# logannye/streaming-zero-knowledge-proofs

Hardware: AMD Instinct MI355X
Metric: STARK prove field-elements/sec (NTT+FRI+Merkle), 2^24 domain, 1/2/4/8 GPUs (higher is better)
Workload: dtype u64; 1 GPU; stark-v1 prove, T=2^21 rows (N=2^24 LDE domain), b=512, tau=8, trace resident in HBM when the timed region starts, proof bytes on the host (host_to_proof beside it: every proof uploads its own trace over PCIe); T=2097152, N=16777216, tau=8, b=512, proof_bytes=2301655, proofs_in_flight_per_gpu=3, upload_bytes_per_proof=69206016, parallelism=replicas x1, 3 independent proofs in flight per GPU

## Files before the change

### include/sezkp_stark.h

```cpp
#ifndef SEZKP_STARK_H
#define SEZKP_STARK_H

#include <stddef.h>
#include <stdint.h>

#ifdef __cplusplus
extern "C" {
#endif

#define SEZKP_ABI_VERSION 4u

#define SEZKP_OK 0
#define SEZKP_E_INVALID (-1)
#define SEZKP_E_DEVICE (-2)
#define SEZKP_E_NOMEM (-3)
#define SEZKP_E_DECODE (-4)
#define SEZKP_E_VERIFY (-5)

#define SEZKP_FLAG_STREAMING 1u

uint32_t sezkp_abi_version(void);
const char* sezkp_version(void);

typedef struct sezkp_buf {
// ... 51 lines not shown
                              size_t err_len);
int32_t sezkp_ctx_wait(sezkp_ctx* ctx, const uint8_t** data, size_t* len, char* err, size_t err_len);
void* sezkp_ctx_stream(const sezkp_ctx* ctx);
typedef struct sezkp_dict_plan_info {
  uint32_t col;
  uint32_t kind;
  uint32_t tape;
  int32_t K;
  uint32_t a;
  uint32_t delta;
  uint32_t R;
  uint32_t dR;
  int64_t min;
} sezkp_dict_plan_info;
int32_t sezkp_ctx_dict_plans(const sezkp_ctx* ctx, sezkp_dict_plan_info* out, int32_t max);

#define SEZKP_AIR_FAMILIES 5
typedef struct sezkp_air_family {
  uint64_t cells, rows, first_row;
  uint32_t first_tape, pad;
  uint64_t first_value;
} sezkp_air_family;
typedef struct sezkp_air_audit {
  uint64_t n_rows;
  uint32_t tau, pad;
  uint64_t rows_violating, first_violating, rows_rejectable, first_rejectable;
  sezkp_air_family fam[SEZKP_AIR_FAMILIES];
} sezkp_air_audit;
int32_t sezkp_ctx_air_audit(sezkp_ctx* ctx, sezkp_air_audit* out, uint8_t* violating_bits, uint8_t* rejectable_bits,
                            char* err, size_t err_len);
// ... 72 lines not shown
```

### streaming-zero-knowledge-proofs_amd/csrc/prover.cpp

```cpp
#include <hip/hip_runtime.h>
#include <stdio.h>
#include <stdlib.h>
#include <string.h>

#include <algorithm>
#include <chrono>
#include <condition_variable>
#include <map>
#include <memory>
#include <mutex>
#include <string>
#include <thread>
#include <vector>

#include "../../include/sezkp_stark.h"
#include "codec.h"
#include "comm.h"
#include "host_crypto.h"
#include "sezkp_internal.h"

using namespace sezkp;

namespace {

// ... 154 lines not shown
  int n_tab_cols = 0;
  uint64_t tab_units = 0;
  uint32_t* d_work = nullptr;
  int n_work = 0;
  uint32_t* d_pw_cols = nullptr;
  int n_pw_cols = 0;
  uint32_t* d_pw_chunks = nullptr;
  int n_pw_chunks = 0;
  DictCol* d_dcols = nullptr;
  int n_dict = 0;
  int64_t* d_dpart = nullptr;
  DictPlan* d_dplans = nullptr;
  std::vector<sezkp_dict_plan_info> dict_info;
  bool have_plans = false;
  uint32_t* d_dtabs = nullptr;
  uint32_t* d_dlev = nullptr;
  std::vector<uint32_t> dict_of;
  uint32_t* d_outer = nullptr;
  uint32_t* d_err = nullptr;
  uint64_t outer_stride = 0;
  uint32_t* d_colroots = nullptr;
  uint64_t* d_base = nullptr;
  ComposeTerms Tm{};
  uint64_t *d_dq_part = nullptr, *d_dq_rlo = nullptr, *d_dq_rhi = nullptr, *d_dq_rhk = nullptr;
  uint64_t* d_lde = nullptr;
  uint64_t* d_fri = nullptr;
  uint32_t* d_roots = nullptr;
  DevChal* d_chal = nullptr;
  DevChal* h_chal = nullptr;
  uint32_t* d_dict_of = nullptr;
// ... 165 lines not shown
    if (async) {
      {
        std::unique_lock<std::mutex> lk(async->mu);
        async->cv.wait(lk, [&] { return async->state != AsyncSlot::RUNNING; });
        async->stop = true;
      }
      async->cv.notify_all();
      if (async->th.joinable()) async->th.join();
    }
    if (st) (void)hipStreamSynchronize(st);
    if (st2) (void)hipStreamSynchronize(st2);
    if (stc) (void)hipStreamSynchronize(stc);
    free_all();
    release_spares();
    free_audit();
    if (h_audit) (void)hipHostFree(h_audit);
    for (auto& e : ev)
      if (e) (void)hipEventDestroy(e);
    for (auto& e : coll_ev) (void)hipEventDestroy(e);
    for (auto& e : kev)
      if (e) (void)hipEventDestroy(e);
    for (auto& e : oev)
      if (e) (void)hipEventDestroy(e);
    if (st2) (void)hipStreamSynchronize(st2);
    if (ev_fold) (void)hipEventDestroy(ev_fold);
    if (ev_tail) (void)hipEventDestroy(ev_tail);
    if (ev_expand) (void)hipEventDestroy(ev_expand);
    if (ev_cols) (void)hipEventDestroy(ev_cols);
    if (ev_qin) (void)hipEventDestroy(ev_qin);
    if (ev_qout) (void)hipEventDestroy(ev_qout);
// ... 238 lines not shown
      for (uint32_t j = k; j < nblk && v.step_start[j] < c1; j++)
        if (j == 0 || v.step_start[j] != v.step_start[j - 1]) inside++;
      if (ch < ch_lo || ch >= ch_hi) continue;
      if (inside <= 16) pw_chunks.push_back((uint32_t)ch);
      else dense_chunk[ch] = 1;
    }
  }
  for (int c = 0; c < ncols; c++) {
    if (use_dict && kind_dict(tm[c].kind)) continue;
    const bool pw = kind_piecewise(tm[c].kind);
    for (uint64_t ch = ch_lo; ch < ch_hi; ch++)
      if (!pw || dense_chunk[ch]) { work.push_back((uint32_t)c); work.push_back((uint32_t)ch); }
  }
  d_tmpl = dalloc<ColTemplate>(ncols);
  up(d_tmpl, tm.data(), tm.size());
  d_colroots = dalloc<uint32_t>((size_t)ncols * 8 + 16);
  d_err = d_colroots + (size_t)ncols * 8;
  HIP_OR_THROW(hipMemset(d_err, 0, 64));
  d_tabs = dalloc<uint32_t>(tab_nodes * 8 + 8);
  n_tab_cols = (int)tab_cols.size();
  d_tab_cols = dalloc<uint32_t>(tab_cols.size() + 1);
  up(d_tab_cols, tab_cols.data(), tab_cols.size());
  for (DictCol& h : dcols)
    if (tm[h.col].kind == 6)
      for (size_t i = 0; i < dcols.size(); i++)
        if (tm[dcols[i].col].kind == 3 && tm[dcols[i].col].tape == tm[h.col].tape) h.mv = (uint32_t)i;
  n_dict = (int)dcols.size();
  have_plans = false;
  dict_info.assign(dcols.size(), sezkp_dict_plan_info{});
  for (size_t i = 0; i < dcols.size(); i++) {
    dict_info[i].col = dcols[i].col;
    dict_info[i].kind = tm[dcols[i].col].kind;
    dict_info[i].tape = tm[dcols[i].col].tape;
  }
  d_dcols = dalloc<DictCol>(dcols.size() + 1);
  up(d_dcols, dcols.data(), dcols.size());
  d_dpart = dalloc<int64_t>(2 * dcols.size() * ((n + 4095) / 4096) + 2);
  d_dplans = dalloc<DictPlan>(dcols.size() + 1);
  d_dtabs = dalloc<uint32_t>(dcols.size() * DICT_LEVELS * DICT_CAP * 8 + 8);
  d_dlev = dalloc<uint32_t>(dcols.size() * (n >> COL_CHUNK_LOG2) * DLEV_NODES * 8 + 8);
  dict_of.assign(ncols, NO_DICT);
  for (size_t i = 0; i < dcols.size(); i++) dict_of[dcols[i].col] = (uint32_t)i;
  n_pw_cols = (int)pw_cols.size();
  d_pw_cols = dalloc<uint32_t>(pw_cols.size() + 1);
  up(d_pw_cols, pw_cols.data(), pw_cols.size());
  n_pw_chunks = (int)pw_chunks.size();
  d_pw_chunks = dalloc<uint32_t>(pw_chunks.size() + 1);
  up(d_pw_chunks, pw_chunks.data(), pw_chunks.size());
  n_work = (int)(work.size() / 2);
  d_work = dalloc<uint32_t>(work.size() + 2);
  up(d_work, work.data(), work.size());
  outer_stride = tree_stored_nodes(logChunks, 0);
  d_outer = dalloc<uint32_t>((size_t)ncols * outer_stride * 8);

// ... 149 lines not shown
    PL.nq = NUM_QUERIES;
    PL.k = k;
    PL.tau = tau;
    PL.open_bytes = 80 + 32 * (uint64_t)logn;
    PL.q_bytes = 16 + PL.open_per_q * PL.open_bytes;
    PL.fr_off = 8 + NUM_QUERIES * PL.q_bytes;
    PL.fq_off = PL.fr_off + 8 + 32 * (uint64_t)(k + 1);
    PL.fq_bytes = 8 + 8 * (uint64_t)(k + 1) + 8;
    for (int r = 0; r < k; r++) PL.fq_bytes += 2 * (16 + 32 * (uint64_t)(k - r));
    PL.tail_off = PL.fq_off + 8 + NUM_QUERIES * PL.fq_bytes;
    PL.total = PL.tail_off + 8 + 32;
    PL.base = dalloc<uint32_t>(PL.total / 4 + 2);
    h_proof = halloc<uint8_t>(hdr_bytes + PL.total);
    memcpy(h_proof, w.b.data(), hdr_bytes);
  }
  h_small = halloc<uint32_t>((size_t)(ncols + k + 2) * 8);
  d_chal = dalloc<DevChal>(1);
  h_chal = halloc<DevChal>(1);
  d_dict_of = dalloc<uint32_t>((size_t)ncols);
  up(d_dict_of, dict_of.data(), dict_of.size());
  if (k > FS_MAX_BETAS) throw Err{SEZKP_E_INVALID, "LDE domain too large for the challenge record"};
  release_spares();
  loaded = true;
}

void sezkp_ctx::alloc_slot(TraceSlot& t) {
  const size_t cells = (size_t)tau * n, nt = (size_t)tau * nblk;
  t.imv = dalloc<int8_t>(n);
  t.mv = dalloc<int8_t>(cells);
  t.wf = dalloc<uint8_t>(cells);
  t.ws = dalloc<uint16_t>(cells);
// ... 273 lines not shown
  const bool no_deep_poly = getenv("SEZKP_NO_DEEP_POLY") != nullptr;
  uint32_t dict_tab_cap = DICT_CAP;
  if (const char* cap = getenv("SEZKP_DICT_TAB_CAP")) {
    const long v = atol(cap);
    if (v >= 1 && v <= (long)DICT_CAP) dict_tab_cap = (uint32_t)v;
  }
  uint64_t dict_plan_rows = 0;
  if (const char* pr = getenv("SEZKP_TEST_DICT_PLAN_ROWS_LOG")) {
    long v = atol(pr);
    int lg = 0;
    while ((2ULL << lg) <= row_hi - row_lo) lg++;
    const long v_max = lg >= 16 ? 40 : 20 + (lg > 14 ? lg - 14 : 0);
    if (v > v_max) v = v_max;
    if (v >= COL_CHUNK_LOG2 && v <= 40) dict_plan_rows = 1ULL << v;
  }
  const int nguard = sharded ? comm->world : 1;
  auto check_guards = [&](const uint32_t* g_h, int ng) {
    for (int r = 0; r < ng; r++) {
      const uint32_t g = g_h[r];
      if (g) {
        const hipError_t me = hipMemsetAsync(d_err, 0, 64, st);
        if (me != hipSuccess) {
          broken = true;
          throw Err{SEZKP_E_DEVICE, std::string("guard word tripped (code ") + std::to_string(g) +
                                        ") and clearing it failed: " + hipGetErrorString(me) +
                                        "; the context is unusable"};
        }
      }
      const std::string who = " on rank " + std::to_string(sharded ? r : rank);
      if (g & GUARD_HEAD_RANGE) throw Err{SEZKP_E_INVALID, head_range_msg(who)};
// ... 13 lines not shown
  size_t nf = 0, no = 0;

  auto enqueue_A = [&]() {
    rec(0);
    ok(launch_expand(st, T, blk_lo, blk_cnt, d_err), "expand");
    rec(1);
    HIP_OR_THROW(hipEventRecord(ev_expand, st));
    HIP_OR_THROW(hipStreamWaitEvent(st2, ev_expand, 0));
    ok(launch_col_tables(st2, T, d_tmpl, d_tab_cols, n_tab_cols, tab_units, d_tabs, blk_lo, blk_cnt), "col_tables");
    ok(launch_col_commit(st2, T, d_tmpl, d_work, n_work, d_tabs, d_outer, outer_stride), "col_commit");
    ok(launch_col_commit_pw(st2, T, d_tmpl, d_pw_cols, n_pw_cols, d_pw_chunks, n_pw_chunks, d_tabs, d_outer,
                            outer_stride, d_err), "col_commit_pw");
    ok(launch_compose_terms(st2, T, Tm, row_lo, row_hi - row_lo), "compose_terms");
    HIP_OR_THROW(hipEventRecord(ev_cols, st2));
    ok(launch_dict_commit(st, T, d_tmpl, d_dcols, n_dict, d_dpart, d_dplans, d_dtabs, d_outer, outer_stride, row_lo,
                          row_hi - row_lo, d_dlev, dict_tab_cap, dict_plan_rows),
       "col_commit_dict");
    HIP_OR_THROW(hipStreamWaitEvent(st, ev_cols, 0));
    static const char* trip = getenv("SEZKP_DEBUG_TRIP_GUARD");
    if (trip && atoi(trip) == rank) HIP_OR_THROW(hipMemsetAsync(d_err, 0x7f, 1, st));
    if (sharded) {
      const size_t bytes = (size_t)(ch_hi - ch_lo) * 32;
      coll("col_chunk_roots", P1 * (bytes * ncols + 4), [&] {
        comm->group_start();
        for (int c = 0; c < ncols; c++) {
          uint32_t* lvl0 = d_outer + (size_t)c * outer_stride * 8;
          comm->allgather(lvl0 + ch_lo * 8, lvl0, bytes, st);
        }
        comm->allgather(d_err, d_err + 8, 4, st);
        comm->group_end();
      });
    }
    rec(2);
    TreeDev outer0{d_outer, d_colroots, logChunks, 0};
    ok(launch_tree_upper(st, &outer0, ncols, outer_stride, 8, 0), "col_outer");
    rec(3);
    HIP_OR_THROW(hipMemcpyAsync(h_small, d_colroots, (size_t)ncols * 32 + 4 * (gofs + nguard), hipMemcpyDeviceToHost,
                                st));
  };
  auto host_1 = [&]() {
    const uint32_t* colroots_h = h_small;
    check_guards(h_small + 8 * ncols + gofs, nguard);
    std::vector<uint8_t> colroots((const uint8_t*)colroots_h, (const uint8_t*)colroots_h + (size_t)ncols * 32);
    for (int c = 0; c < ncols; c++) memcpy(h_proof + root_pos[c], colroots.data() + 32 * c, 32);

    tr.absorb("manifest_root", mroot, 32);
    tr.absorb_u64("n", n);
    tr.absorb_u64("tau", tau);
    tr.absorb_u64("n_cols", (uint64_t)ncols);
    for (int c = 0; c < ncols; c++) tr.absorb("col_root", colroots.data() + 32 * c, 32);
    mark("tr_roots");
    auto ab = tr.challenge("alphas", 64);
    uint64_t a[8];
    for (int i = 0; i < 8; i++) a[i] = rd64(ab.data() + 8 * i) % GL_P_HOST;
    tr.absorb("masks", "masks", 5);
    tr.absorb_u64("n_masks", 1);
    tr.absorb_u64("deg", 4);
// ... 370 lines not shown
  for (int q = 0; q < NUM_QUERIES; q++) {
    const uint64_t at = PL.fq_off + 8 + q * PL.fq_bytes;
    put64(at, (uint64_t)k + 1);
    for (int r = 0; r <= k; r++) put64(at + 8 + 8 * r, pos[(size_t)q * (k + 1) + r]);
    put64(at + 8 + 8 * (uint64_t)(k + 1), (uint64_t)k);
  }
  memcpy(body + PL.tail_off, h_small + 8 * (k + 1), 8);
  memcpy(body + PL.tail_off + 8, mroot, 32);
  const size_t out = hdr_bytes + PL.total;
  const auto t_end = clk::now();
  host_ms[0] = std::chrono::duration<double, std::milli>(t_end - t_enter).count();
  host_ms[1] = t_sync;
  host_ms[2] = t_last;
  host_ms[3] = std::chrono::duration<double, std::milli>(t_end - t_ser).count();
  have_plans = true;
  return out;
}

extern "C" {

uint32_t sezkp_abi_version(void) { return SEZKP_ABI_VERSION; }
const char* sezkp_version(void) { return "sezkp-mi355x 0.1.0 (stark-v1, gfx950)"; }

void sezkp_buf_free(sezkp_buf* b) {
  if (b && b->data) {
    free(b->data);
    b->data = nullptr;
    b->len = 0;
  }
}
// ... 287 lines not shown
      hipMemcpy(pl.data(), ctx->d_dplans, (size_t)cnt * sizeof(DictPlan), hipMemcpyDeviceToHost) != hipSuccess) {
    (void)hipGetLastError();
    return SEZKP_E_DEVICE;
  }
  for (int32_t i = 0; i < cnt; i++) {
    sezkp_dict_plan_info& o = out[i];
    o = ctx->dict_info[(size_t)i];
    o.K = pl[i].K;
    o.a = pl[i].a;
    o.delta = pl[i].delta;
    o.R = pl[i].R;
    o.dR = pl[i].delta ? pl[i].dR : 0;
    o.min = pl[i].min;
  }
  return cnt;
}
int32_t sezkp_ctx_comm_stats(const sezkp_ctx* ctx, sezkp_comm_stat* out, int32_t max) {
  if (!ctx || !out || max <= 0) return 0;
  int32_t cnt = 0;
  for (const auto& c : ctx->coll_stats) {
    if (cnt >= max) break;
    sezkp_comm_stat& o = out[cnt++];
    memset(o.name, 0, sizeof o.name);
    strncpy(o.name, c.name, sizeof o.name - 1);
    o.bytes = c.bytes;
    float ms = 0;
    o.ms = hipEventElapsedTime(&ms, c.a, c.b) == hipSuccess ? ms : -1.0;
  }
  (void)hipGetLastError();
  return cnt;
// ... 450 lines not shown
```

### streaming-zero-knowledge-proofs_amd/csrc/sezkp_internal.h

```cpp
#pragma once
#include <hip/hip_runtime.h>
#include <stddef.h>
#include <stdint.h>

#include <vector>

namespace sezkp {

struct DevChal;
struct ComposeTerms;

struct NttTables {
  const uint64_t* hi;
  const uint64_t* lo;
  const uint64_t* p3_hi;
  const uint64_t* p3_lo;
  int K;
  int S;
};

struct NttPassArgs {
  uint64_t* a;
  const uint64_t* src;
  NttTables tw;
// ... 136 lines not shown
struct DictCol {
  uint32_t col;
  uint32_t mv;
  uint64_t tab;
};
struct DictPlan {
  int64_t min;
  uint32_t R;
  int32_t K;
  uint32_t pw[DICT_LEVELS];
  uint32_t delta;
  int64_t dmin;
  uint32_t dR;
  uint32_t a;
};
__host__ __device__ inline bool kind_dict(uint32_t kind) { return kind == 0 || (kind >= 3 && kind <= 6); }
constexpr int DICT_LANE_LOG = 6;
constexpr int DLEV_NODES = 30;
__host__ __device__ inline int dlev_base(int level) { return level == 6 ? 0 : level == 7 ? 16 : level == 8 ? 24 : 28; }
constexpr uint32_t NO_DICT = 0xFFFFFFFFu;
__host__ __device__ inline int dict_extra(int K) { return K >= 3 ? 2 : (K == 2 ? 1 : 0); }
constexpr int OPEN_REQ_WORDS = 5;

constexpr int LSTORE_FRI = 6;
constexpr int COL_CHUNK_LOG2 = 10;
struct ProofLayout {
  uint32_t* base;
  uint64_t open_bytes;
  uint64_t q_bytes;
  uint64_t fr_off, fq_off, fq_bytes, tail_off, total;
// ... 11 lines not shown
  uint64_t K3;
  uint64_t beta[FS_MAX_BETAS];
};

hipError_t launch_trace_image(hipStream_t st, const int8_t* raw_mv, const uint8_t* raw_hw, const uint16_t* raw_ws,
                              uint64_t n, int tau, int8_t* mv, uint8_t* wf, uint16_t* ws, uint64_t r0 = 0,
                              uint64_t r1 = ~0ull);
hipError_t launch_expand(hipStream_t st, const TraceDev& T, uint32_t blk_lo, uint32_t blk_cnt, uint32_t* d_err);
hipError_t launch_col_tables(hipStream_t st, const TraceDev& T, const ColTemplate* d_tmpl, const uint32_t* d_tab_cols,
                             int n_tab_cols, uint64_t tab_entries, uint32_t* tabs, uint32_t blk_lo, uint32_t blk_cnt);
hipError_t launch_col_commit(hipStream_t st, const TraceDev& T, const ColTemplate* d_tmpl, const uint32_t* d_work,
                             int nwork, const uint32_t* tabs, uint32_t* outer_nodes, uint64_t outer_stride_nodes);
hipError_t launch_dict_commit(hipStream_t st, const TraceDev& T, const ColTemplate* d_tmpl, const DictCol* d_dcols,
                              int ndict, int64_t* d_part, DictPlan* d_plans, uint32_t* d_dtabs, uint32_t* outer_nodes,
                              uint64_t outer_stride_nodes, uint64_t row0, uint64_t nrows, uint32_t* d_dlev,
                              uint32_t tab_cap = DICT_CAP, uint64_t plan_rows = 0);
hipError_t launch_dict_prepare(hipStream_t st, const TraceDev& T, const ColTemplate* d_tmpl, const DictCol* d_dcols,
                               int ndict, int64_t* d_part, DictPlan* d_plans, uint64_t row0, uint64_t nrows,
                               uint32_t tab_cap = DICT_CAP, uint64_t plan_rows = 0);
hipError_t launch_dict_levels(hipStream_t st, const ColTemplate* d_tmpl, const DictCol* d_dcols, int ndict,
                              const DictPlan* d_plans, uint32_t* d_dtabs, int lvl_lo, int lvl_hi);
hipError_t launch_dict_commit_cols(hipStream_t st, const TraceDev& T, const ColTemplate* d_tmpl,
                                   const DictCol* d_dcols, int ndict, const DictPlan* d_plans,
                                   const uint32_t* d_dtabs, uint32_t* outer_nodes, uint64_t outer_stride_nodes,
                                   uint64_t row0, uint64_t nrows, uint32_t* d_dlev, int kmin, int kmax);
hipError_t launch_col_commit_pw(hipStream_t st, const TraceDev& T, const ColTemplate* d_tmpl, const uint32_t* d_pw_cols,
                                int n_pw_cols, const uint32_t* d_chunks, int nchunks, const uint32_t* tabs,
                                uint32_t* outer_nodes, uint64_t outer_stride_nodes, uint32_t* d_err);
hipError_t launch_compose_terms(hipStream_t st, const TraceDev& T, const ComposeTerms& Tm, uint64_t row0,
                                uint64_t nrows);
hipError_t launch_compose_combine(hipStream_t st, const ComposeTerms& Tm, const DevChal* ch, const NttTables& tw,
                                  int logn, uint64_t* out, uint64_t row0, uint64_t nrows);
hipError_t launch_deep(hipStream_t st, uint64_t* y, int logN, uint64_t z, const NttTables& tw, int logP = 0,
                       uint32_t g = 0, uint64_t shift = 3);
hipError_t launch_scale_pow_bitrev(hipStream_t st, uint64_t* a, int logn, uint64_t base, uint64_t* scratch);
hipError_t launch_fold_any(hipStream_t st, const uint64_t* in, uint64_t* out, uint64_t n_out, uint64_t beta);
hipError_t launch_leaves_u64(hipStream_t st, const uint64_t* v, uint64_t n, uint32_t* out);
hipError_t launch_leaves_labeled(hipStream_t st, const uint64_t* v, uint64_t n, const ColTemplate& ct, uint32_t* out);
hipError_t launch_merkle_level(hipStream_t st, const uint32_t* in, uint64_t len, uint32_t* out);
struct MerkleLevels {
// ... 88 lines not shown
```

### streaming-zero-knowledge-proofs_amd/csrc/trace.hip

```cpp
#include <type_traits>

#include "dev_common.h"
#include "col_leaf.h"
#include "sezkp_internal.h"
#include "compose.h"

namespace sezkp {

constexpr int TR_THREADS = 256;

__global__ void __launch_bounds__(TR_THREADS) k_trace_image(const int8_t* __restrict__ raw_mv,
                                                          const uint8_t* __restrict__ raw_hw,
                                                          const uint16_t* __restrict__ raw_ws, uint64_t n, int tau,
                                                          int8_t* __restrict__ mv, uint8_t* __restrict__ wf,
                                                          uint16_t* __restrict__ ws, uint64_t r0, uint64_t r1) {
  const uint64_t s = r0 + (uint64_t)blockIdx.x * TR_THREADS + threadIdx.x;
  if (s >= r1) return;
  const size_t i0 = (size_t)s * tau;
  for (int r = 0; r < tau; r++) {
    const size_t o = (size_t)r * n + s;
    const bool w = raw_hw[i0 + r] != 0;
    mv[o] = raw_mv[i0 + r];
    wf[o] = w ? 1 : 0;
    ws[o] = w ? raw_ws[i0 + r] : 0;
// ... 1354 lines not shown
  if ((tid & 63) == 0) { slo[tid >> 6] = lo; shi[tid >> 6] = hi; }
  __syncthreads();
  if (tid == 0) {
    for (int w = 1; w < TR_THREADS / 64; w++) {
      lo = slo[w] < lo ? slo[w] : lo;
      hi = shi[w] > hi ? shi[w] : hi;
    }
    int64_t* o = part + 2 * ((uint64_t)blockIdx.y * nparts + blockIdx.x);
    o[0] = lo;
    o[1] = hi;
  }
}

__global__ void __launch_bounds__(TR_THREADS) k_dict_plan(const int64_t* __restrict__ part, uint32_t nparts,
                                                          uint64_t n, uint64_t nrows, const DictCol* __restrict__ dcols,
                                                          DictPlan* __restrict__ plans, uint32_t tab_cap) {
  __shared__ int64_t slo[TR_THREADS / 64], shi[TR_THREADS / 64];
  int64_t lo, hi, mlo = 0, mhi = -1;
  reduce_parts(part + 2 * (uint64_t)blockIdx.x * nparts, nparts, lo, hi, slo, shi);
  const uint32_t mvc = dcols[blockIdx.x].mv;
  if (mvc != NO_DICT) reduce_parts(part + 2 * (uint64_t)mvc * nparts, nparts, mlo, mhi, slo, shi);
  if (threadIdx.x == 0) plans[blockIdx.x] = make_plan(lo, hi, mvc != NO_DICT, mlo, mhi, n, nrows, tab_cap);
}

__device__ __forceinline__ void dict_entry(const ColTemplate& ct, const DictCol& dc, const DictPlan& P, uint32_t S,
                                           uint32_t* __restrict__ tabs, int lvl, uint32_t e) {
  uint32_t* tl = tabs + 8 * (dc.tab + (uint64_t)lvl * DICT_CAP);
  uint32_t h[8];
  if (lvl == 2 && P.delta) {
    const uint32_t* t1 = tl - 8 * (uint64_t)DICT_CAP;
    const int64_t R = P.R, dR = P.dR;
    int64_t c[4];
    c[0] = e % R;
    int64_t rest = e / R;
    bool ok = true;
#pragma unroll
    for (int j = 1; j < 4; j++) {
// ... 11 lines not shown
  } else {
    const uint32_t* tp = tl - 8 * (uint64_t)DICT_CAP;
    uint32_t a[8], b[8];
    node_load(tp + 8 * (uint64_t)(e % S), a);
    node_load(tp + 8 * (uint64_t)(e / S), b);
    b3_parent(a, b, h);
  }
  node_store(tl + 8 * (uint64_t)e, h);
}

constexpr int DICT_FLAT_MAX = 1024;
constexpr int DICT_FLAT_WGS = 2048;
__global__ void __launch_bounds__(TR_THREADS) k_dict_level(const ColTemplate* __restrict__ tmpl,
                                                           const DictCol* __restrict__ dcols,
                                                           const DictPlan* __restrict__ plans,
                                                           uint32_t* __restrict__ tabs, int ndict, int lvl) {
  __shared__ uint32_t off[DICT_FLAT_MAX + 1];
  const int tid = threadIdx.x;
  for (int c = tid; c < ndict; c += TR_THREADS) {
    const DictPlan& P = plans[c];
    uint32_t size = 0;
#pragma unroll
    for (int k = 0; k < DICT_LEVELS; k++)
      if (k == lvl && lvl <= P.K) size = P.pw[k];
    off[c + 1] = size;
  }
  __syncthreads();
  if (tid == 0) {
    off[0] = 0;
    for (int c = 0; c < ndict; c++) off[c + 1] += off[c];
  }
  __syncthreads();
  const uint32_t total = off[ndict];
  for (uint32_t g = blockIdx.x * TR_THREADS + tid; g < total; g += gridDim.x * TR_THREADS) {
    int lo = 0, hi = ndict;
    while (hi - lo > 1) {
      const int mid = (lo + hi) >> 1;
      if (off[mid] <= g) lo = mid;
      else hi = mid;
    }
// ... 132 lines not shown
}
hipError_t launch_col_tables(hipStream_t st, const TraceDev& T, const ColTemplate* d_tmpl, const uint32_t* d_tab_cols,
                             int n_tab_cols, uint64_t max_units, uint32_t* tabs, uint32_t blk_lo, uint32_t blk_cnt) {
  if (n_tab_cols == 0) return hipSuccess;
  if ((uint64_t)blk_lo + blk_cnt > T.nblk) return hipErrorInvalidValue;
  const unsigned gx = (unsigned)((max_units + TR_THREADS - 1) / TR_THREADS);
  hipLaunchKernelGGL(k_col_tables, dim3(gx, n_tab_cols), dim3(TR_THREADS), 0, st, T, d_tmpl, d_tab_cols, tabs, blk_lo,
                     blk_cnt);
  return hipGetLastError();
}
static hipError_t dict_shape_ok(const TraceDev& T, uint64_t row0, uint64_t nrows) {
  if (T.n < (1ULL << COL_CHUNK_LOG2)) return hipErrorInvalidValue;
  if (row0 + nrows > T.n || (nrows != T.n && (row0 % DICT_WG_ROWS || nrows % DICT_WG_ROWS))) return hipErrorInvalidValue;
  return hipSuccess;
}
hipError_t launch_dict_prepare(hipStream_t st, const TraceDev& T, const ColTemplate* d_tmpl, const DictCol* d_dcols,
                               int ndict, int64_t* d_part, DictPlan* d_plans, uint64_t row0, uint64_t nrows,
                               uint32_t tab_cap, uint64_t plan_rows) {
  if (ndict == 0) return hipSuccess;
  hipError_t e = dict_shape_ok(T, row0, nrows);
  if (e != hipSuccess) return e;
  if (tab_cap == 0 || tab_cap > DICT_CAP) return hipErrorInvalidValue;
  const int sweeps = (int)std::max<uint64_t>(1, std::min<uint64_t>(8, nrows / (64ull * DICT_RANGE_STEP)));
  const uint64_t prow = (uint64_t)sweeps * DICT_RANGE_STEP;
  const uint32_t nparts = (uint32_t)((nrows + prow - 1) / prow);
  hipLaunchKernelGGL(k_dict_range, dim3(nparts, ndict), dim3(TR_THREADS), 0, st, T, d_tmpl, d_dcols, d_part, nparts,
                     row0, row0 + nrows, sweeps);
  if ((e = hipGetLastError()) != hipSuccess) return e;
  hipLaunchKernelGGL(k_dict_plan, dim3(ndict), dim3(TR_THREADS), 0, st, d_part, nparts, T.n,
                     plan_rows ? plan_rows : nrows, d_dcols, d_plans, tab_cap);
  return hipGetLastError();
}
hipError_t launch_dict_levels(hipStream_t st, const ColTemplate* d_tmpl, const DictCol* d_dcols, int ndict,
                              const DictPlan* d_plans, uint32_t* d_dtabs, int lvl_lo, int lvl_hi) {
  if (lvl_lo < 0 || lvl_hi > DICT_LEVELS) return hipErrorInvalidValue;
  for (int l = lvl_lo; l < lvl_hi; l++) {
    for (int c0 = 0; c0 < ndict; c0 += DICT_FLAT_MAX) {
      const int nc = ndict - c0 < DICT_FLAT_MAX ? ndict - c0 : DICT_FLAT_MAX;
      hipLaunchKernelGGL(k_dict_level, dim3(DICT_FLAT_WGS), dim3(TR_THREADS), 0, st, d_tmpl, d_dcols + c0,
                         d_plans + c0, d_dtabs, nc, l);
      hipError_t e = hipGetLastError();
      if (e != hipSuccess) return e;
    }
  }
  return hipSuccess;
}
hipError_t launch_dict_commit_cols(hipStream_t st, const TraceDev& T, const ColTemplate* d_tmpl,
                                   const DictCol* d_dcols, int ndict, const DictPlan* d_plans,
                                   const uint32_t* d_dtabs, uint32_t* outer_nodes, uint64_t outer_stride_nodes,
                                   uint64_t row0, uint64_t nrows, uint32_t* d_dlev, int kmin, int kmax) {
  if (ndict == 0) return hipSuccess;
  hipError_t e = dict_shape_ok(T, row0, nrows);
  if (e != hipSuccess) return e;
  const uint64_t wg_rows = (uint64_t)DICT_WG_LANES << DICT_LANE_LOG;
  const unsigned gx = (unsigned)((nrows + wg_rows - 1) / wg_rows);
  hipLaunchKernelGGL(k_col_commit_dict, dim3(gx, ndict), dim3(DICT_WG_LANES), 0, st, T, d_tmpl, d_dcols, d_plans, d_dtabs,
                     outer_nodes, outer_stride_nodes, row0, row0 + nrows, d_dlev, kmin, kmax);
  return hipGetLastError();
}
hipError_t launch_dict_commit(hipStream_t st, const TraceDev& T, const ColTemplate* d_tmpl, const DictCol* d_dcols,
                              int ndict, int64_t* d_part, DictPlan* d_plans, uint32_t* d_dtabs, uint32_t* outer_nodes,
                              uint64_t outer_stride_nodes, uint64_t row0, uint64_t nrows, uint32_t* d_dlev,
                              uint32_t tab_cap, uint64_t plan_rows) {
  hipError_t e = launch_dict_prepare(st, T, d_tmpl, d_dcols, ndict, d_part, d_plans, row0, nrows, tab_cap, plan_rows);
  if (e == hipSuccess && ndict) e = launch_dict_levels(st, d_tmpl, d_dcols, ndict, d_plans, d_dtabs, 0, DICT_LEVELS);
  if (e == hipSuccess)
    e = launch_dict_commit_cols(st, T, d_tmpl, d_dcols, ndict, d_plans, d_dtabs, outer_nodes, outer_stride_nodes, row0,
                                nrows, d_dlev, -1, DICT_LEVELS);
  return e;
}

hipError_t launch_col_commit(hipStream_t st, const TraceDev& T, const ColTemplate* d_tmpl, const uint32_t* d_work,
                             int nwork, const uint32_t* tabs, uint32_t* outer_nodes, uint64_t outer_stride_nodes) {
  if (nwork == 0) return hipSuccess;
  hipLaunchKernelGGL(k_col_commit, dim3(nwork), dim3(TR_THREADS), 0, st, T, d_tmpl, d_work, tabs, outer_nodes,
                     outer_stride_nodes);
  return hipGetLastError();
}
hipError_t launch_col_commit_pw(hipStream_t st, const TraceDev& T, const ColTemplate* d_tmpl, const uint32_t* d_pw_cols,
                                int n_pw_cols, const uint32_t* d_chunks, int nchunks, const uint32_t* tabs,
// ... 60 lines not shown
```

### streaming-zero-knowledge-proofs_amd/sezkp_amd/_lib.py

```python
from __future__ import annotations

import ctypes as C
import os

PKG_ROOT = os.path.dirname(os.path.dirname(os.path.abspath(__file__)))
LIB_PATH = os.path.join(PKG_ROOT, "lib", "libsezkp_stark.so")

SEZKP_OK = 0
SEZKP_E_INVALID = -1
SEZKP_E_DEVICE = -2
SEZKP_E_NOMEM = -3
SEZKP_E_DECODE = -4
SEZKP_E_VERIFY = -5
SEZKP_FLAG_STREAMING = 1
ABI_VERSION = 4

EXPORTS = [
    "sezkp_abi_version", "sezkp_version", "sezkp_buf_free", "sezkp_stark_v1_prove",
    "sezkp_stark_v1_prove_artifact_cbor", "sezkp_stark_v1_verify", "sezkp_ctx_create", "sezkp_ctx_destroy",
    "sezkp_ctx_upload", "sezkp_ctx_prove", "sezkp_ctx_stage_times", "sezkp_ctx_stream", "sezkp_gl_ntt",
    "sezkp_gl_coset_lde_deep", "sezkp_fri_fold_commit", "sezkp_merkle_root_u64", "sezkp_manifest_root",
    "sezkp_blocks_decode_cbor", "sezkp_blocks_view", "sezkp_blocks_free", "sezkp_blake3",
    "sezkp_comm_unique_id", "sezkp_ctx_create_sharded", "sezkp_ctx_create_sharded_host", "sezkp_ctx_prove_borrow",
    "sezkp_blocks_decode_jsonl", "sezkp_blocks_encode_jsonl", "sezkp_manifest_decode", "sezkp_ctx_dist_ntt",
    "sezkp_blocks_encode_cbor", "sezkp_simulate_trace", "sezkp_simulate_blocks",
    "sezkp_ctx_prove_async", "sezkp_ctx_wait", "sezkp_ctx_stage", "sezkp_host_register", "sezkp_host_unregister",
    "sezkp_fri_fold", "sezkp_blake3_leaves_u64", "sezkp_blake3_leaves_labeled", "sezkp_merkle_node_count",
    "sezkp_merkle_build", "sezkp_merkle_paths", "sezkp_manifest_frontier_root", "sezkp_ctx_comm_stats",
    "sezkp_fs_xof", "sezkp_ctx_upload_rows", "sezkp_shard_rows", "sezkp_blocks_decode_jsonl_meta",
    "sezkp_blocks_line_offsets", "sezkp_manifest_leaf_hashes", "sezkp_merkle_root_of_leaves",
    "sezkp_ctx_create_sharded_solo", "sezkp_blocks_decode_jsonl_lines", "sezkp_ctx_dict_plans",
    "sezkp_ctx_air_audit", "sezkp_stark_v1_air_audit",
]

AIR_FAMILIES = ("mv_domain", "head_range", "slack_range", "sym_range", "boundary")


class AirFamilyC(C.Structure):
    _fields_ = [("cells", C.c_uint64), ("rows", C.c_uint64), ("first_row", C.c_uint64), ("first_tape", C.c_uint32),
                ("pad", C.c_uint32), ("first_value", C.c_uint64)]


class AirAuditC(C.Structure):
    _fields_ = [("n_rows", C.c_uint64), ("tau", C.c_uint32), ("pad", C.c_uint32), ("rows_violating", C.c_uint64),
                ("first_violating", C.c_uint64), ("rows_rejectable", C.c_uint64), ("first_rejectable", C.c_uint64),
                ("fam", AirFamilyC * len(AIR_FAMILIES))]

# ... 63 lines not shown
    L.sezkp_stark_v1_prove.argtypes = [C.POINTER(BlockView), C.c_char_p, C.c_uint32, C.POINTER(Buf), C.POINTER(Buf)] + E
    L.sezkp_stark_v1_prove_artifact_cbor.argtypes = [C.POINTER(BlockView), C.c_char_p, C.c_uint32, C.POINTER(Buf)] + E
    L.sezkp_stark_v1_verify.argtypes = [C.c_char_p, C.c_size_t, C.POINTER(BlockView), C.c_char_p] + E
    L.sezkp_ctx_create.restype = C.c_void_p
    L.sezkp_ctx_create.argtypes = [C.c_int32] + E
    L.sezkp_ctx_destroy.argtypes = [C.c_void_p]
    L.sezkp_ctx_upload.argtypes = [C.c_void_p, C.POINTER(BlockView)] + E
    L.sezkp_ctx_prove.argtypes = [C.c_void_p, C.c_char_p, C.c_uint32, C.POINTER(Buf)] + E
    L.sezkp_ctx_prove_borrow.argtypes = [C.c_void_p, C.c_char_p, C.c_uint32, C.POINTER(C.POINTER(C.c_uint8)),
                                         C.POINTER(C.c_size_t)] + E
    L.sezkp_ctx_stage_times.argtypes = [C.c_void_p, C.POINTER(C.c_double), C.c_int32]
    L.sezkp_ctx_stream.restype = C.c_void_p
    L.sezkp_ctx_comm_stats.argtypes = [C.c_void_p, C.POINTER(CommStat), C.c_int32]
    L.sezkp_ctx_stream.argtypes = [C.c_void_p]
    L.sezkp_ctx_dict_plans.argtypes = [C.c_void_p, C.POINTER(DictPlanInfo), C.c_int32]
    L.sezkp_gl_ntt.argtypes = [C.c_void_p, C.c_void_p, C.c_uint32, C.c_int32, C.c_void_p]
    L.sezkp_gl_coset_lde_deep.argtypes = [C.c_void_p, C.c_uint32, C.c_uint32, C.c_uint64, C.c_uint64, C.c_void_p,
                                          C.c_void_p, C.c_void_p]
    L.sezkp_fri_fold.argtypes = [C.c_void_p, C.c_uint64, C.c_uint64, C.c_void_p, C.c_void_p]
    L.sezkp_blake3_leaves_u64.argtypes = [C.c_void_p, C.c_uint64, C.c_void_p, C.c_void_p]
    L.sezkp_blake3_leaves_labeled.argtypes = [C.c_void_p, C.c_uint64, C.c_char_p, C.c_uint32, C.c_void_p, C.c_void_p]
    L.sezkp_merkle_node_count.restype = C.c_uint64
    L.sezkp_merkle_node_count.argtypes = [C.c_uint64]
    L.sezkp_merkle_build.argtypes = [C.c_void_p, C.c_uint64, C.c_void_p, C.c_void_p]
    L.sezkp_merkle_paths.argtypes = [C.c_void_p, C.c_uint64, C.c_void_p, C.c_uint32, C.c_void_p, C.c_void_p]
    L.sezkp_fri_fold_commit.argtypes = [C.c_void_p, C.c_uint64, C.c_uint64, C.c_void_p, C.c_char_p, C.c_void_p]
    L.sezkp_merkle_root_u64.argtypes = [C.c_void_p, C.c_uint64, C.c_char_p, C.c_void_p]
    L.sezkp_manifest_root.argtypes = [C.POINTER(BlockView), C.c_char_p]
    L.sezkp_manifest_frontier_root.argtypes = [C.POINTER(BlockView), C.c_char_p]
    L.sezkp_blocks_decode_cbor.argtypes = [C.c_char_p, C.c_size_t, C.POINTER(C.c_void_p)] + E
# ... 54 lines not shown
```

### streaming-zero-knowledge-proofs_amd/sezkp_amd/backend.py

```python
from __future__ import annotations

import ctypes as C
import json
import struct
from dataclasses import dataclass, field

from ._lib import AIR_FAMILIES, SEZKP_FLAG_STREAMING, AirAuditC, Buf, SezkpError, check, lib, take_buf
from .blocks import BlockSoA

STAGES = ["expand", "col_commit", "col_outer", "compose", "intt", "lde_ntt", "deep", "layer0_tree",
          "layer0_upper", "fri_fold_trees", "col_openings", "fri_paths", "total",
          "host_wall", "host_sync_wait", "host_final_wait", "host_serialize",
          "k_forest16"]


@dataclass
class ProofArtifact:
    backend: str
    manifest_root: bytes
    proof_bytes: bytes
    meta: dict = field(default_factory=dict)

    def to_cbor(self) -> bytes:
        out = bytearray(b"\xa4")
# ... 213 lines not shown
            b, ms = int(buf[i].bytes), float(buf[i].ms)
            out.append({"name": buf[i].name.decode(), "bytes": b, "ms": ms,
                        "GBs": (b / ms / 1e6) if ms > 0 else None})
        return out

    def dict_plans(self) -> list:
        from ._lib import DictPlanInfo
        cap = 1 + 4 * self.tau
        buf = (DictPlanInfo * cap)()
        n = lib.sezkp_ctx_dict_plans(self._h, buf, cap)
        if n < 0:
            why = {-1: "a proof is in flight on this context (or the context is closed)",
                   -2: "copying the plans from the device failed"}.get(n, "unexpected return code")
            raise SezkpError(n, f"dict_plans: {why}")
        return [{f: int(getattr(buf[i], f)) for f, _ in DictPlanInfo._fields_} for i in range(n)]

    def dist_ntt(self, local, scratch=None, inverse: bool = False, sync: bool = True):
        import torch
        if local.dtype not in (torch.int64, torch.uint64) or not local.is_cuda or not local.is_contiguous():
            raise SezkpError(-1, "local must be a contiguous 64-bit device tensor")
        m = local.numel()
        if m & (m - 1):
            raise SezkpError(-1, "local length must be a power of two")
        if scratch is None:
            scratch = torch.empty_like(local)
        log_n = (m * self.world).bit_length() - 1
        if sync:
            torch.cuda.current_stream(local.device).synchronize()
        err = C.create_string_buffer(1024)
        check(lib.sezkp_ctx_dist_ntt(self._h, local.data_ptr(), scratch.data_ptr(), log_n, -1 if inverse else 1,
# ... 50 lines not shown
```

Measured before the change: 9.673 billion field-elements/s.

## Cache dictionary lookup tables on device across proofs keyed by column value ranges

Keeps per-column dictionary tables allocated for the life of the context instead of reallocating them for every proof. A device-side key (value range, mv range, epoch) is checked in the plan kernel, and the level kernels skip columns, or whole levels, whose tables are unchanged. Host-side epochs invalidate the cache when the shape, row window or plan parameters change, and an env var can disable it. It adds a small stats readback and a new API for cache hit counts, and risks stale tables if the key misses some input that the tables depend on.

```diff
diff --git a/include/sezkp_stark.h b/include/sezkp_stark.h
--- a/include/sezkp_stark.h
+++ b/include/sezkp_stark.h
@@ -89,6 +89,8 @@
   int64_t min;
 } sezkp_dict_plan_info;
 int32_t sezkp_ctx_dict_plans(const sezkp_ctx* ctx, sezkp_dict_plan_info* out, int32_t max);
+int32_t sezkp_ctx_dict_cache_stats(const sezkp_ctx* ctx, uint32_t* cols_rebuilt, uint32_t* cols_reused,
+                                   uint64_t* entries_rebuilt);
 
 #define SEZKP_AIR_FAMILIES 5
 typedef struct sezkp_air_family {
diff --git a/streaming-zero-knowledge-proofs_amd/csrc/prover.cpp b/streaming-zero-knowledge-proofs_amd/csrc/prover.cpp
--- a/streaming-zero-knowledge-proofs_amd/csrc/prover.cpp
+++ b/streaming-zero-knowledge-proofs_amd/csrc/prover.cpp
@@ -192,6 +192,30 @@
   std::vector<sezkp_dict_plan_info> dict_info;
   bool have_plans = false;
   uint32_t* d_dtabs = nullptr;
+  DictKey* d_dkeys = nullptr;
+  uint64_t* d_dlvl_seq = nullptr;
+  uint32_t* d_dreuse = nullptr;
+  uint32_t* d_dstatus = nullptr;
+  size_t dict_cache_cols = ~(size_t)0;
+  uint64_t dict_epoch = 1, dict_seq = 0;
+  struct DictHostKey {
+    uint64_t n = 0, nrows = 0, row0 = 0, plan_rows = 0;
+    uint32_t tab_cap = 0;
+    bool operator==(const DictHostKey& o) const {
+      return n == o.n && nrows == o.nrows && row0 == o.row0 && plan_rows == o.plan_rows && tab_cap == o.tab_cap;
+    }
+  } dict_hkey;
+  std::vector<uint8_t> dict_shape;
+  bool dict_dirty = false;
+  uint32_t dstat_rebuilt = 0, dstat_reused = 0;
+  uint64_t dstat_entries = 0;
+  void free_dict_cache() {
+    if (d_dtabs) (void)hipFree(d_dtabs);
+    if (d_dkeys) (void)hipFree(d_dkeys);
+    d_dtabs = nullptr;
+    d_dkeys = nullptr;
+    dict_cache_cols = ~(size_t)0;
+  }
   uint32_t* d_dlev = nullptr;
   std::vector<uint32_t> dict_of;
   uint32_t* d_outer = nullptr;
@@ -387,6 +411,7 @@
     free_all();
     release_spares();
     free_audit();
+    free_dict_cache();
     if (h_audit) (void)hipHostFree(h_audit);
     for (auto& e : ev)
       if (e) (void)hipEventDestroy(e);
@@ -655,8 +680,9 @@
   }
   d_tmpl = dalloc<ColTemplate>(ncols);
   up(d_tmpl, tm.data(), tm.size());
-  d_colroots = dalloc<uint32_t>((size_t)ncols * 8 + 16);
+  d_colroots = dalloc<uint32_t>((size_t)ncols * 8 + 16 + 2 * dcols.size());
   d_err = d_colroots + (size_t)ncols * 8;
+  d_dstatus = d_err + 16;
   HIP_OR_THROW(hipMemset(d_err, 0, 64));
   d_tabs = dalloc<uint32_t>(tab_nodes * 8 + 8);
   n_tab_cols = (int)tab_cols.size();
@@ -678,7 +704,31 @@
   up(d_dcols, dcols.data(), dcols.size());
   d_dpart = dalloc<int64_t>(2 * dcols.size() * ((n + 4095) / 4096) + 2);
   d_dplans = dalloc<DictPlan>(dcols.size() + 1);
-  d_dtabs = dalloc<uint32_t>(dcols.size() * DICT_LEVELS * DICT_CAP * 8 + 8);
+  if (dcols.size() != dict_cache_cols) {
+    free_dict_cache();
+    dict_epoch++;
+    const size_t nd = dcols.size();
+    const size_t key_bytes = nd * sizeof(DictKey) + DICT_LEVELS * 8, cache_bytes = key_bytes + nd * 4 + 64;
+    HIP_OR_THROW(hipMalloc((void**)&d_dtabs, (nd * DICT_LEVELS * DICT_CAP * 8 + 8) * sizeof(uint32_t)));
+    HIP_OR_THROW(hipMalloc((void**)&d_dkeys, cache_bytes));
+    HIP_OR_THROW(hipMemset(d_dkeys, 0, cache_bytes));
+    d_dlvl_seq = reinterpret_cast<uint64_t*>(d_dkeys + nd);
+    d_dreuse = reinterpret_cast<uint32_t*>(d_dlvl_seq + DICT_LEVELS);
+    dict_cache_cols = nd;
+  }
+  {
+    std::vector<uint8_t> shape(dcols.size() * (sizeof(ColTemplate) + sizeof(DictCol)));
+    uint8_t* p = shape.data();
+    for (const DictCol& d : dcols) {
+      memcpy(p, &tm[d.col], sizeof(ColTemplate));
+      memcpy(p + sizeof(ColTemplate), &d, sizeof(DictCol));
+      p += sizeof(ColTemplate) + sizeof(DictCol);
+    }
+    if (shape != dict_shape) {
+      dict_shape.swap(shape);
+      dict_epoch++;
+    }
+  }
   d_dlev = dalloc<uint32_t>(dcols.size() * (n >> COL_CHUNK_LOG2) * DLEV_NODES * 8 + 8);
   dict_of.assign(ncols, NO_DICT);
   for (size_t i = 0; i < dcols.size(); i++) dict_of[dcols[i].col] = (uint32_t)i;
@@ -858,7 +908,7 @@
     h_proof = halloc<uint8_t>(hdr_bytes + PL.total);
     memcpy(h_proof, w.b.data(), hdr_bytes);
   }
-  h_small = halloc<uint32_t>((size_t)(ncols + k + 2) * 8);
+  h_small = halloc<uint32_t>((size_t)(ncols + k + 4) * 8 + 2 * (size_t)n_dict);
   d_chal = dalloc<DevChal>(1);
   h_chal = halloc<DevChal>(1);
   d_dict_of = dalloc<uint32_t>((size_t)ncols);
@@ -1162,6 +1212,23 @@
     if (v > v_max) v = v_max;
     if (v >= COL_CHUNK_LOG2 && v <= 40) dict_plan_rows = 1ULL << v;
   }
+  {
+    const char* dce = getenv("SEZKP_DICT_CACHE");
+    const bool cache_off = dce && atoi(dce) == 0;
+    DictHostKey hk;
+    hk.n = n;
+    hk.nrows = row_hi - row_lo;
+    hk.row0 = row_lo;
+    hk.plan_rows = dict_plan_rows;
+    hk.tab_cap = dict_tab_cap;
+    if (cache_off || dict_dirty || !(hk == dict_hkey)) dict_epoch++;
+    dict_hkey = hk;
+    dict_dirty = true;
+    dict_seq++;
+  }
+  const DictCache dcache{d_dkeys, d_dreuse, d_dlvl_seq, d_dstatus, dict_epoch, dict_seq};
+  uint32_t st_rebuilt = 0;
+  uint64_t st_entries = 0;
   const int nguard = sharded ? comm->world : 1;
   auto check_guards = [&](const uint32_t* g_h, int ng) {
     for (int r = 0; r < ng; r++) {
@@ -1205,10 +1272,10 @@
     ok(launch_compose_terms(st2, T, Tm, row_lo, row_hi - row_lo), "compose_terms");
     HIP_OR_THROW(hipEventRecord(ev_cols, st2));
     ok(launch_dict_commit(st, T, d_tmpl, d_dcols, n_dict, d_dpart, d_dplans, d_dtabs, d_outer, outer_stride, row_lo,
-                          row_hi - row_lo, d_dlev, dict_tab_cap, dict_plan_rows),
+                          row_hi - row_lo, d_dlev, dcache, dict_tab_cap, dict_plan_rows),
        "col_commit_dict");
     HIP_OR_THROW(hipStreamWaitEvent(st, ev_cols, 0));
-    static const char* trip = getenv("SEZKP_DEBUG_TRIP_GUARD");
+    const char* trip = getenv("SEZKP_DEBUG_TRIP_GUARD");
     if (trip && atoi(trip) == rank) HIP_OR_THROW(hipMemsetAsync(d_err, 0x7f, 1, st));
     if (sharded) {
       const size_t bytes = (size_t)(ch_hi - ch_lo) * 32;
@@ -1226,12 +1293,18 @@
     TreeDev outer0{d_outer, d_colroots, logChunks, 0};
     ok(launch_tree_upper(st, &outer0, ncols, outer_stride, 8, 0), "col_outer");
     rec(3);
-    HIP_OR_THROW(hipMemcpyAsync(h_small, d_colroots, (size_t)ncols * 32 + 4 * (gofs + nguard), hipMemcpyDeviceToHost,
-                                st));
+    HIP_OR_THROW(hipMemcpyAsync(h_small, d_colroots,
+                                n_dict ? (size_t)ncols * 32 + 4 * (16 + 2 * (size_t)n_dict)
+                                       : (size_t)ncols * 32 + 4 * (gofs + nguard),
+                                hipMemcpyDeviceToHost, st));
   };
   auto host_1 = [&]() {
     const uint32_t* colroots_h = h_small;
     check_guards(h_small + 8 * ncols + gofs, nguard);
+    for (int c = 0; c < n_dict; c++) {
+      st_rebuilt += h_small[8 * ncols + 16 + 2 * c];
+      st_entries += h_small[8 * ncols + 16 + 2 * c + 1];
+    }
     std::vector<uint8_t> colroots((const uint8_t*)colroots_h, (const uint8_t*)colroots_h + (size_t)ncols * 32);
     for (int c = 0; c < ncols; c++) memcpy(h_proof + root_pos[c], colroots.data() + 32 * c, 32);
 
@@ -1632,6 +1705,10 @@
   host_ms[2] = t_last;
   host_ms[3] = std::chrono::duration<double, std::milli>(t_end - t_ser).count();
   have_plans = true;
+  dict_dirty = false;
+  dstat_rebuilt = st_rebuilt;
+  dstat_reused = (uint32_t)n_dict - st_rebuilt;
+  dstat_entries = st_entries;
   return out;
 }
 
@@ -1949,6 +2026,17 @@
     o.min = pl[i].min;
   }
   return cnt;
+}
+int32_t sezkp_ctx_dict_cache_stats(const sezkp_ctx* cctx, uint32_t* cols_rebuilt, uint32_t* cols_reused,
+                                   uint64_t* entries_rebuilt) {
+  sezkp_ctx* ctx = const_cast<sezkp_ctx*>(cctx);
+  if (!ctx || !cols_rebuilt || !cols_reused || !entries_rebuilt) return SEZKP_E_INVALID;
+  if (ctx->busy()) return SEZKP_E_INVALID;
+  const bool have = ctx->loaded && ctx->have_plans && ctx->n_dict != 0;
+  *cols_rebuilt = have ? ctx->dstat_rebuilt : 0;
+  *cols_reused = have ? ctx->dstat_reused : 0;
+  *entries_rebuilt = have ? ctx->dstat_entries : 0;
+  return SEZKP_OK;
 }
 int32_t sezkp_ctx_comm_stats(const sezkp_ctx* ctx, sezkp_comm_stat* out, int32_t max) {
   if (!ctx || !out || max <= 0) return 0;
diff --git a/streaming-zero-knowledge-proofs_amd/csrc/sezkp_internal.h b/streaming-zero-knowledge-proofs_amd/csrc/sezkp_internal.h
--- a/streaming-zero-knowledge-proofs_amd/csrc/sezkp_internal.h
+++ b/streaming-zero-knowledge-proofs_amd/csrc/sezkp_internal.h
@@ -174,6 +174,18 @@
   uint32_t dR;
   uint32_t a;
 };
+struct DictKey {
+  int64_t lo, hi, mlo, mhi;
+  uint64_t epoch;
+};
+struct DictCache {
+  DictKey* keys;
+  uint32_t* reuse;
+  uint64_t* lvl_seq;
+  uint32_t* status;
+  uint64_t epoch;
+  uint64_t seq;
+};
 __host__ __device__ inline bool kind_dict(uint32_t kind) { return kind == 0 || (kind >= 3 && kind <= 6); }
 constexpr int DICT_LANE_LOG = 6;
 constexpr int DLEV_NODES = 30;
@@ -215,16 +227,7 @@
 hipError_t launch_dict_commit(hipStream_t st, const TraceDev& T, const ColTemplate* d_tmpl, const DictCol* d_dcols,
                               int ndict, int64_t* d_part, DictPlan* d_plans, uint32_t* d_dtabs, uint32_t* outer_nodes,
                               uint64_t outer_stride_nodes, uint64_t row0, uint64_t nrows, uint32_t* d_dlev,
-                              uint32_t tab_cap = DICT_CAP, uint64_t plan_rows = 0);
-hipError_t launch_dict_prepare(hipStream_t st, const TraceDev& T, const ColTemplate* d_tmpl, const DictCol* d_dcols,
-                               int ndict, int64_t* d_part, DictPlan* d_plans, uint64_t row0, uint64_t nrows,
-                               uint32_t tab_cap = DICT_CAP, uint64_t plan_rows = 0);
-hipError_t launch_dict_levels(hipStream_t st, const ColTemplate* d_tmpl, const DictCol* d_dcols, int ndict,
-                              const DictPlan* d_plans, uint32_t* d_dtabs, int lvl_lo, int lvl_hi);
-hipError_t launch_dict_commit_cols(hipStream_t st, const TraceDev& T, const ColTemplate* d_tmpl,
-                                   const DictCol* d_dcols, int ndict, const DictPlan* d_plans,
-                                   const uint32_t* d_dtabs, uint32_t* outer_nodes, uint64_t outer_stride_nodes,
-                                   uint64_t row0, uint64_t nrows, uint32_t* d_dlev, int kmin, int kmax);
+                              const DictCache& dc, uint32_t tab_cap = DICT_CAP, uint64_t plan_rows = 0);
 hipError_t launch_col_commit_pw(hipStream_t st, const TraceDev& T, const ColTemplate* d_tmpl, const uint32_t* d_pw_cols,
                                 int n_pw_cols, const uint32_t* d_chunks, int nchunks, const uint32_t* tabs,
                                 uint32_t* outer_nodes, uint64_t outer_stride_nodes, uint32_t* d_err);
diff --git a/streaming-zero-knowledge-proofs_amd/csrc/trace.hip b/streaming-zero-knowledge-proofs_amd/csrc/trace.hip
--- a/streaming-zero-knowledge-proofs_amd/csrc/trace.hip
+++ b/streaming-zero-knowledge-proofs_amd/csrc/trace.hip
@@ -1392,13 +1392,31 @@
 
 __global__ void __launch_bounds__(TR_THREADS) k_dict_plan(const int64_t* __restrict__ part, uint32_t nparts,
                                                           uint64_t n, uint64_t nrows, const DictCol* __restrict__ dcols,
-                                                          DictPlan* __restrict__ plans, uint32_t tab_cap) {
+                                                          DictPlan* __restrict__ plans, uint32_t tab_cap, DictCache dc) {
   __shared__ int64_t slo[TR_THREADS / 64], shi[TR_THREADS / 64];
   int64_t lo, hi, mlo = 0, mhi = -1;
   reduce_parts(part + 2 * (uint64_t)blockIdx.x * nparts, nparts, lo, hi, slo, shi);
   const uint32_t mvc = dcols[blockIdx.x].mv;
   if (mvc != NO_DICT) reduce_parts(part + 2 * (uint64_t)mvc * nparts, nparts, mlo, mhi, slo, shi);
-  if (threadIdx.x == 0) plans[blockIdx.x] = make_plan(lo, hi, mvc != NO_DICT, mlo, mhi, n, nrows, tab_cap);
+  if (threadIdx.x == 0) {
+    const DictPlan P = make_plan(lo, hi, mvc != NO_DICT, mlo, mhi, n, nrows, tab_cap);
+    plans[blockIdx.x] = P;
+    DictKey* key = dc.keys + blockIdx.x;
+    const DictKey old = *key;
+    const bool same = old.lo == lo && old.hi == hi && old.mlo == mlo && old.mhi == mhi && old.epoch == dc.epoch;
+    uint32_t entries = 0;
+    if (!same) {
+      *key = DictKey{lo, hi, mlo, mhi, dc.epoch};
+#pragma unroll
+      for (int k = 0; k < DICT_LEVELS; k++) {
+        entries += P.pw[k];
+        if (P.pw[k]) dc.lvl_seq[k] = dc.seq;
+      }
+    }
+    dc.reuse[blockIdx.x] = same ? 1u : 0u;
+    dc.status[2 * blockIdx.x] = same ? 0u : 1u;
+    dc.status[2 * blockIdx.x + 1] = entries;
+  }
 }
 
 __device__ __forceinline__ void dict_entry(const ColTemplate& ct, const DictCol& dc, const DictPlan& P, uint32_t S,
@@ -1440,7 +1458,10 @@
 __global__ void __launch_bounds__(TR_THREADS) k_dict_level(const ColTemplate* __restrict__ tmpl,
                                                            const DictCol* __restrict__ dcols,
                                                            const DictPlan* __restrict__ plans,
+                                                           const uint32_t* __restrict__ reuse,
+                                                           const uint64_t* __restrict__ lvl_seq, uint64_t seq,
                                                            uint32_t* __restrict__ tabs, int ndict, int lvl) {
+  if (lvl_seq[lvl] != seq) return;
   __shared__ uint32_t off[DICT_FLAT_MAX + 1];
   const int tid = threadIdx.x;
   for (int c = tid; c < ndict; c += TR_THREADS) {
@@ -1449,7 +1470,7 @@
 #pragma unroll
     for (int k = 0; k < DICT_LEVELS; k++)
       if (k == lvl && lvl <= P.K) size = P.pw[k];
-    off[c + 1] = size;
+    off[c + 1] = reuse[c] ? 0 : size;
   }
   __syncthreads();
   if (tid == 0) {
@@ -1612,9 +1633,10 @@
   if (row0 + nrows > T.n || (nrows != T.n && (row0 % DICT_WG_ROWS || nrows % DICT_WG_ROWS))) return hipErrorInvalidValue;
   return hipSuccess;
 }
-hipError_t launch_dict_prepare(hipStream_t st, const TraceDev& T, const ColTemplate* d_tmpl, const DictCol* d_dcols,
-                               int ndict, int64_t* d_part, DictPlan* d_plans, uint64_t row0, uint64_t nrows,
-                               uint32_t tab_cap, uint64_t plan_rows) {
+static hipError_t launch_dict_prepare(hipStream_t st, const TraceDev& T, const ColTemplate* d_tmpl,
+                                      const DictCol* d_dcols, int ndict, int64_t* d_part, DictPlan* d_plans,
+                                      uint64_t row0, uint64_t nrows, uint32_t tab_cap, uint64_t plan_rows,
+                                      const DictCache& dc) {
   if (ndict == 0) return hipSuccess;
   hipError_t e = dict_shape_ok(T, row0, nrows);
   if (e != hipSuccess) return e;
@@ -1626,27 +1648,28 @@
                      row0, row0 + nrows, sweeps);
   if ((e = hipGetLastError()) != hipSuccess) return e;
   hipLaunchKernelGGL(k_dict_plan, dim3(ndict), dim3(TR_THREADS), 0, st, d_part, nparts, T.n,
-                     plan_rows ? plan_rows : nrows, d_dcols, d_plans, tab_cap);
+                     plan_rows ? plan_rows : nrows, d_dcols, d_plans, tab_cap, dc);
   return hipGetLastError();
 }
-hipError_t launch_dict_levels(hipStream_t st, const ColTemplate* d_tmpl, const DictCol* d_dcols, int ndict,
-                              const DictPlan* d_plans, uint32_t* d_dtabs, int lvl_lo, int lvl_hi) {
+static hipError_t launch_dict_levels(hipStream_t st, const ColTemplate* d_tmpl, const DictCol* d_dcols, int ndict,
+                                     const DictPlan* d_plans, const DictCache& dc, uint32_t* d_dtabs, int lvl_lo,
+                                     int lvl_hi) {
   if (lvl_lo < 0 || lvl_hi > DICT_LEVELS) return hipErrorInvalidValue;
   for (int l = lvl_lo; l < lvl_hi; l++) {
     for (int c0 = 0; c0 < ndict; c0 += DICT_FLAT_MAX) {
       const int nc = ndict - c0 < DICT_FLAT_MAX ? ndict - c0 : DICT_FLAT_MAX;
       hipLaunchKernelGGL(k_dict_level, dim3(DICT_FLAT_WGS), dim3(TR_THREADS), 0, st, d_tmpl, d_dcols + c0,
-                         d_plans + c0, d_dtabs, nc, l);
+                         d_plans + c0, dc.reuse + c0, dc.lvl_seq, dc.seq, d_dtabs, nc, l);
       hipError_t e = hipGetLastError();
       if (e != hipSuccess) return e;
     }
   }
   return hipSuccess;
 }
-hipError_t launch_dict_commit_cols(hipStream_t st, const TraceDev& T, const ColTemplate* d_tmpl,
-                                   const DictCol* d_dcols, int ndict, const DictPlan* d_plans,
-                                   const uint32_t* d_dtabs, uint32_t* outer_nodes, uint64_t outer_stride_nodes,
-                                   uint64_t row0, uint64_t nrows, uint32_t* d_dlev, int kmin, int kmax) {
+static hipError_t launch_dict_commit_cols(hipStream_t st, const TraceDev& T, const ColTemplate* d_tmpl,
+                                          const DictCol* d_dcols, int ndict, const DictPlan* d_plans,
+                                          const uint32_t* d_dtabs, uint32_t* outer_nodes, uint64_t outer_stride_nodes,
+                                          uint64_t row0, uint64_t nrows, uint32_t* d_dlev, int kmin, int kmax) {
   if (ndict == 0) return hipSuccess;
   hipError_t e = dict_shape_ok(T, row0, nrows);
   if (e != hipSuccess) return e;
@@ -1659,9 +1682,11 @@
 hipError_t launch_dict_commit(hipStream_t st, const TraceDev& T, const ColTemplate* d_tmpl, const DictCol* d_dcols,
                               int ndict, int64_t* d_part, DictPlan* d_plans, uint32_t* d_dtabs, uint32_t* outer_nodes,
                               uint64_t outer_stride_nodes, uint64_t row0, uint64_t nrows, uint32_t* d_dlev,
-                              uint32_t tab_cap, uint64_t plan_rows) {
-  hipError_t e = launch_dict_prepare(st, T, d_tmpl, d_dcols, ndict, d_part, d_plans, row0, nrows, tab_cap, plan_rows);
-  if (e == hipSuccess && ndict) e = launch_dict_levels(st, d_tmpl, d_dcols, ndict, d_plans, d_dtabs, 0, DICT_LEVELS);
+                              const DictCache& dc, uint32_t tab_cap, uint64_t plan_rows) {
+  hipError_t e =
+      launch_dict_prepare(st, T, d_tmpl, d_dcols, ndict, d_part, d_plans, row0, nrows, tab_cap, plan_rows, dc);
+  if (e == hipSuccess && ndict)
+    e = launch_dict_levels(st, d_tmpl, d_dcols, ndict, d_plans, dc, d_dtabs, 0, DICT_LEVELS);
   if (e == hipSuccess)
     e = launch_dict_commit_cols(st, T, d_tmpl, d_dcols, ndict, d_plans, d_dtabs, outer_nodes, outer_stride_nodes, row0,
                                 nrows, d_dlev, -1, DICT_LEVELS);
diff --git a/streaming-zero-knowledge-proofs_amd/sezkp_amd/_lib.py b/streaming-zero-knowledge-proofs_amd/sezkp_amd/_lib.py
--- a/streaming-zero-knowledge-proofs_amd/sezkp_amd/_lib.py
+++ b/streaming-zero-knowledge-proofs_amd/sezkp_amd/_lib.py
@@ -30,7 +30,7 @@
     "sezkp_fs_xof", "sezkp_ctx_upload_rows", "sezkp_shard_rows", "sezkp_blocks_decode_jsonl_meta",
     "sezkp_blocks_line_offsets", "sezkp_manifest_leaf_hashes", "sezkp_merkle_root_of_leaves",
     "sezkp_ctx_create_sharded_solo", "sezkp_blocks_decode_jsonl_lines", "sezkp_ctx_dict_plans",
-    "sezkp_ctx_air_audit", "sezkp_stark_v1_air_audit",
+    "sezkp_ctx_air_audit", "sezkp_stark_v1_air_audit", "sezkp_ctx_dict_cache_stats",
 ]
 
 AIR_FAMILIES = ("mv_domain", "head_range", "slack_range", "sym_range", "boundary")
@@ -124,6 +124,8 @@
     L.sezkp_ctx_comm_stats.argtypes = [C.c_void_p, C.POINTER(CommStat), C.c_int32]
     L.sezkp_ctx_stream.argtypes = [C.c_void_p]
     L.sezkp_ctx_dict_plans.argtypes = [C.c_void_p, C.POINTER(DictPlanInfo), C.c_int32]
+    L.sezkp_ctx_dict_cache_stats.argtypes = [C.c_void_p, C.POINTER(C.c_uint32), C.POINTER(C.c_uint32),
+                                             C.POINTER(C.c_uint64)]
     L.sezkp_gl_ntt.argtypes = [C.c_void_p, C.c_void_p, C.c_uint32, C.c_int32, C.c_void_p]
     L.sezkp_gl_coset_lde_deep.argtypes = [C.c_void_p, C.c_uint32, C.c_uint32, C.c_uint64, C.c_uint64, C.c_void_p,
                                           C.c_void_p, C.c_void_p]
diff --git a/streaming-zero-knowledge-proofs_amd/sezkp_amd/backend.py b/streaming-zero-knowledge-proofs_amd/sezkp_amd/backend.py
--- a/streaming-zero-knowledge-proofs_amd/sezkp_amd/backend.py
+++ b/streaming-zero-knowledge-proofs_amd/sezkp_amd/backend.py
@@ -251,6 +251,13 @@
                    -2: "copying the plans from the device failed"}.get(n, "unexpected return code")
             raise SezkpError(n, f"dict_plans: {why}")
         return [{f: int(getattr(buf[i], f)) for f, _ in DictPlanInfo._fields_} for i in range(n)]
+
+    def dict_cache_stats(self) -> dict:
+        rebuilt, reused, entries = C.c_uint32(0), C.c_uint32(0), C.c_uint64(0)
+        rc = lib.sezkp_ctx_dict_cache_stats(self._h, C.byref(rebuilt), C.byref(reused), C.byref(entries))
+        if rc < 0:
+            raise SezkpError(rc, "dict_cache_stats: a proof is in flight on this context (or the context is closed)")
+        return {"cols_rebuilt": rebuilt.value, "cols_reused": reused.value, "entries_rebuilt": entries.value}
 
     def dist_ntt(self, local, scratch=None, inverse: bool = False, sync: bool = True):
         import torch
```

After: 9.838 billion field-elements/s (median of 6 runs). 1.02x the previous value.
